# BoMingZhao/GaussianPrediction

Hardware: AMD Instinct MI355X
Metric: rendered views/s (full train step) @1M Gaussians 1352x1014 (higher is better)
Workload: dtype f32; 1 GPU; configs[2]: HyperNeRF-like 1M Gaussians, 1352x1014, stage-3 full train step (deform, raster, L1+SSIM loss, Adam: all HIP kernels); gaussians=1000000, width=1352, height=1014, keypoints=250, nearest_num=6, parallelism=view-parallel x1, ranks_seen_by_rccl=1, self_launched=False

## Files before the change

### gaussianprediction_amd/csrc/raster_kernels.hip

```cpp
#include "gp_common.h"
#include "raster_kernels.h"

#define GP_LOG2E 1.4426950408889634f
__device__ static const float SH_C0 = 0.28209479177387814f;
__device__ static const float SH_C1 = 0.4886025119029199f;
__device__ static const float SH_C2[5] = {1.0925484305920792f, -1.0925484305920792f, 0.31539156525252005f,
                                          -1.0925484305920792f, 0.5462742152960396f};
__device__ static const float SH_C3[7] = {-0.5900435899266435f, 2.890611442640554f, -0.4570457994644658f,
                                          0.3731763325901154f, -0.4570457994644658f, 1.445305721320277f,
                                          -0.5900435899266435f};

__device__ __forceinline__ float3 xform4x3(const float* __restrict__ m, float x, float y, float z) {
    float3 o;
    o.x = fmaf(m[0], x, fmaf(m[4], y, fmaf(m[8], z, m[12])));
    o.y = fmaf(m[1], x, fmaf(m[5], y, fmaf(m[9], z, m[13])));
    o.z = fmaf(m[2], x, fmaf(m[6], y, fmaf(m[10], z, m[14])));
    return o;
}
__device__ __forceinline__ float4 xform4x4(const float* __restrict__ m, float x, float y, float z) {
    float4 o;
    o.x = fmaf(m[0], x, fmaf(m[4], y, fmaf(m[8], z, m[12])));
    o.y = fmaf(m[1], x, fmaf(m[5], y, fmaf(m[9], z, m[13])));
    o.z = fmaf(m[2], x, fmaf(m[6], y, fmaf(m[10], z, m[14])));
    o.w = fmaf(m[3], x, fmaf(m[7], y, fmaf(m[11], z, m[15])));
// ... 853 lines not shown
                        if (MODE == 2) ++n_eval;
                        const int off = (int)lst[i];
                        const float4 q0 = *(const float4*)(s_rec + off);
                        const float4 q1 = *(const float4*)(s_rec + off + 16);
                        const float2 q2 = *(const float2*)(s_rec + off + 32);
                        const float dx = q0.x - pxf, dy = q0.y - pyf;
                        const float e = fmaf(dx, fmaf(q0.z, dx, q0.w * dy), fmaf(q1.x * dy, dy, q1.y));
                        if (!(e > q1.y)) {
                            const float alpha = fminf(0.99f, __builtin_amdgcn_exp2f(e));
                            if (!(alpha < 1.f / 255.f)) {
                                const float w = alpha * T;
                                const float test_T = T - w;
                                if (test_T < 0.0001f) {
                                    lim = -1;
                                } else {
                                    const int posv = off + sbase;
                                    C01.x = fmaf(q1.z, w, C01.x);
                                    C01.y = fmaf(q1.w, w, C01.y);
                                    C2D.x = fmaf(q2.x, w, C2D.x);
                                    C2D.y = fmaf(q2.y, w, C2D.y);
                                    if (w > best) { best = w; best_pos = posv; }
                                    T = test_T;
                                    last = posv;
                                    if (MODE == 2) ++n_contr;
                                }
                            }
                        }
                    }
                }
            }
            if (!__any(lim >= 0) && lane == 0) s_done[wave] = 1;
        }
    }
    if (MODE == 2) {
#pragma unroll
        for (int dd = 32; dd >= 1; dd >>= 1) { n_eval += __shfl_xor(n_eval, dd); n_contr += __shfl_xor(n_contr, dd); }
        if (lane == 0) { atomicAdd(&g_pair_counters[0], (unsigned long long)n_contr); atomicAdd(&g_pair_counters[1], (unsigned long long)n_eval); }
    }
    const float C0 = C01.x, C1 = C01.y, C2 = C2D.x, Dp = C2D.y;
    const size_t HW = (size_t)d.H * d.W;
    const int last_n = last < 0 ? 0 : last / CF2_REC + 1;
    if (inside) {
        const size_t pix = (size_t)py * d.W + px;
        out_color[pix] = fmaf(T, bg[0], C0);
        out_color[HW + pix] = fmaf(T, bg[1], C1);
        out_color[2 * HW + pix] = fmaf(T, bg[2], C2);
        out_depth[pix] = Dp;
        out_tidx[pix] = best_pos < 0 ? -1 : (int32_t)point_list[range.x + best_pos / CF2_REC];
        final_T[pix] = T;
        n_contrib[pix] = last_n;
    }
    if (tile_work) {
        int mx = inside ? last_n : 0;
#pragma unroll
        for (int dd = 32; dd >= 1; dd >>= 1) mx = max(mx, __shfl_xor(mx, dd));
        if (lane == 0) s_last[wave] = mx;
        __syncthreads();
        if (tid == 0) tile_work[tile] = max(max(s_last[0], s_last[1]), max(s_last[2], s_last[3]));
    }
}
__global__ __launch_bounds__(CF_THREADS) void gp_composite_fwd_sb_kernel(GP_CF_ARGS) {
    gp_composite_fwd_sb_body<1>(d, ranges, point_list, rec, bg, out_color, out_depth, out_tidx, final_T, n_contrib, order, tile_work, smask);
}
__global__ __launch_bounds__(CF_THREADS) void gp_composite_fwd_sbc_kernel(GP_CF_ARGS) {
    gp_composite_fwd_sb_body<0>(d, ranges, point_list, rec, bg, out_color, out_depth, out_tidx, final_T, n_contrib, order, tile_work, smask);
}
__global__ __launch_bounds__(CF_THREADS) void gp_composite_fwd_count_kernel(GP_CF_ARGS) {
    gp_composite_fwd_sb_body<2>(d, ranges, point_list, rec, bg, out_color, out_depth, out_tidx, final_T, n_contrib, order, tile_work, smask);
}
int gp_pair_counters_read(unsigned long long* out4) {
    if (hipDeviceSynchronize() != hipSuccess) return 1;
    if (hipMemcpyFromSymbol(out4, HIP_SYMBOL(g_pair_counters), 4 * sizeof(unsigned long long)) != hipSuccess) return 1;
    unsigned long long z[4] = {0, 0, 0, 0};
    return hipMemcpyToSymbol(HIP_SYMBOL(g_pair_counters), z, sizeof(z)) == hipSuccess ? 0 : 1;
}

__device__ __forceinline__ void dpp_scan2_add(float& a, float& b) {
    asm volatile(
        "s_nop 1\n\t"
        "v_add_f32_dpp %0, %0, %0 row_shr:1 row_mask:0xf bank_mask:0xf\n\t"
        "v_add_f32_dpp %1, %1, %1 row_shr:1 row_mask:0xf bank_mask:0xf\n\t"
        "s_nop 0\n\t"
        "v_add_f32_dpp %0, %0, %0 row_shr:2 row_mask:0xf bank_mask:0xf\n\t"
        "v_add_f32_dpp %1, %1, %1 row_shr:2 row_mask:0xf bank_mask:0xf\n\t"
        "s_nop 0\n\t"
        "v_add_f32_dpp %0, %0, %0 row_shr:4 row_mask:0xf bank_mask:0xf\n\t"
        "v_add_f32_dpp %1, %1, %1 row_shr:4 row_mask:0xf bank_mask:0xf\n\t"
        "s_nop 0\n\t"
        "v_add_f32_dpp %0, %0, %0 row_shr:8 row_mask:0xf bank_mask:0xf\n\t"
        "v_add_f32_dpp %1, %1, %1 row_shr:8 row_mask:0xf bank_mask:0xf\n\t"
        "s_nop 0\n\t"
        "v_add_f32_dpp %0, %0, %0 row_bcast:15 row_mask:0xa bank_mask:0xf\n\t"
        "v_add_f32_dpp %1, %1, %1 row_bcast:15 row_mask:0xa bank_mask:0xf\n\t"
        "s_nop 0\n\t"
        "v_add_f32_dpp %0, %0, %0 row_bcast:31 row_mask:0xc bank_mask:0xf\n\t"
        "v_add_f32_dpp %1, %1, %1 row_bcast:31 row_mask:0xc bank_mask:0xf\n\t"
        "s_nop 1"
        : "+v"(a), "+v"(b));
}
__device__ __forceinline__ void dpp_scan2_mul(float& a, float& b) {
    asm volatile(
        "s_nop 1\n\t"
        "v_mul_f32_dpp %0, %0, %0 row_shr:1 row_mask:0xf bank_mask:0xf\n\t"
        "v_mul_f32_dpp %1, %1, %1 row_shr:1 row_mask:0xf bank_mask:0xf\n\t"
        "s_nop 0\n\t"
        "v_mul_f32_dpp %0, %0, %0 row_shr:2 row_mask:0xf bank_mask:0xf\n\t"
        "v_mul_f32_dpp %1, %1, %1 row_shr:2 row_mask:0xf bank_mask:0xf\n\t"
        "s_nop 0\n\t"
        "v_mul_f32_dpp %0, %0, %0 row_shr:4 row_mask:0xf bank_mask:0xf\n\t"
        "v_mul_f32_dpp %1, %1, %1 row_shr:4 row_mask:0xf bank_mask:0xf\n\t"
        "s_nop 0\n\t"
        "v_mul_f32_dpp %0, %0, %0 row_shr:8 row_mask:0xf bank_mask:0xf\n\t"
        "v_mul_f32_dpp %1, %1, %1 row_shr:8 row_mask:0xf bank_mask:0xf\n\t"
        "s_nop 0\n\t"
        "v_mul_f32_dpp %0, %0, %0 row_bcast:15 row_mask:0xa bank_mask:0xf\n\t"
        "v_mul_f32_dpp %1, %1, %1 row_bcast:15 row_mask:0xa bank_mask:0xf\n\t"
        "s_nop 0\n\t"
        "v_mul_f32_dpp %0, %0, %0 row_bcast:31 row_mask:0xc bank_mask:0xf\n\t"
        "v_mul_f32_dpp %1, %1, %1 row_bcast:31 row_mask:0xc bank_mask:0xf\n\t"
        "s_nop 1"
        : "+v"(a), "+v"(b));
}



__device__ __forceinline__ void gp_pixpair(const RasterDims& d, int px0, int py, float bg0, float bg1, float bg2,
                                           const float* __restrict__ out_color, const float* __restrict__ out_depth,
                                           const float* __restrict__ final_T, const int32_t* __restrict__ n_contrib,
                                           const float* __restrict__ dL_dpix, const float* __restrict__ dL_dpixdepth, float4* o) {
    const size_t HW = (size_t)d.H * d.W;
    float dl[2][4] = {{0.f, 0.f, 0.f, 0.f}, {0.f, 0.f, 0.f, 0.f}};
    float tb[2] = {0.f, 0.f}, rem[2] = {0.f, 0.f};
    int nc[2] = {0, 0};
#pragma unroll
    for (int u = 0; u < 2; ++u) {
        const int px = px0 + u;
        if (px < d.W && py < d.H) {
            const size_t pix = (size_t)py * d.W + px;
            dl[u][0] = dL_dpix[pix]; dl[u][1] = dL_dpix[HW + pix]; dl[u][2] = dL_dpix[2 * HW + pix];
            dl[u][3] = dL_dpixdepth ? dL_dpixdepth[pix] : 0.f;
            tb[u] = final_T[pix] * (bg0 * dl[u][0] + bg1 * dl[u][1] + bg2 * dl[u][2]);
            rem[u] = out_color[pix] * dl[u][0] + out_color[HW + pix] * dl[u][1] + out_color[2 * HW + pix] * dl[u][2] - tb[u];
            if (dL_dpixdepth) rem[u] += out_depth[pix] * dl[u][3];
            nc[u] = n_contrib[pix];
        }
    }
    o[0] = make_float4(dl[0][0], dl[1][0], dl[0][1], dl[1][1]);
    o[1] = make_float4(dl[0][2], dl[1][2], tb[0], tb[1]);
    o[2] = make_float4(__int_as_float(nc[0]), __int_as_float(nc[1]), rem[0], rem[1]);
    o[3] = make_float4(dl[0][3], dl[1][3], 0.f, 0.f);
}

__device__ int g_bwd_ablate;
int gp_bwd_set_ablate(int v) { return hipMemcpyToSymbol(HIP_SYMBOL(g_bwd_ablate), &v, sizeof(int)) == hipSuccess ? 0 : 1; }

template <bool HAS_DEPTH, int ROWS, int COLS>
__device__ __forceinline__ void gp_composite_bwd_body(RasterDims d, const int2* __restrict__ ranges,
                                                       const uint32_t* __restrict__ point_list, const uint16_t* __restrict__ smask,
                                                       const float4* __restrict__ rec, const float* __restrict__ bg,
                                                       const float* __restrict__ out_color, const float* __restrict__ out_depth,
                                                       const float* __restrict__ final_T, const int32_t* __restrict__ n_contrib,
                                                       const float* __restrict__ dL_dpix, const float* __restrict__ dL_dpixdepth,
                                                       float* __restrict__ g_mean2D,
                                                       float* __restrict__ g_conic, float* __restrict__ g_opacity,
                                                       float* __restrict__ g_color, float* __restrict__ g_depth,
                                                       const uint32_t* __restrict__ order) {
    constexpr int PAIRS = ROWS * COLS / 2;
    static_assert(PAIRS <= 64, "one lane per pixel pair in the prologue");
    __shared__ float4 s_pp[PAIRS][4];
    __shared__ float2 s_dd[HAS_DEPTH ? PAIRS : 1];
    constexpr int parts_x = GP_TILE / COLS, parts = (GP_TILE / ROWS) * parts_x;
    const int xcd = blockIdx.x & 7, jw = blockIdx.x >> 3;
    const int slot = (jw / parts) * 8 + xcd;
    const int part = jw % parts;
    if (slot >= d.gx * d.gy) return;
    const int tile = __builtin_amdgcn_readfirstlane(order ? (int)order[slot] : slot);
    const int tx = tile % d.gx, ty = tile / d.gx;
    const int lane = threadIdx.x;
    const int2 range = ranges[tile];
    int max_nc;
    {
        max_nc = 0;
        if (lane < PAIRS) {
            float4 me[4];
            gp_pixpair(d, tx * GP_TILE + (part % parts_x) * COLS + 2 * (lane % (COLS / 2)), ty * GP_TILE + (part / parts_x) * ROWS + lane / (COLS / 2),
                       bg[0], bg[1], bg[2], out_color, out_depth, final_T, n_contrib, dL_dpix, HAS_DEPTH ? dL_dpixdepth : nullptr, me);
            const float4 t0 = me[0], t1 = me[1], t = me[2];
            s_pp[lane][1] = t0; s_pp[lane][2] = t1;
            s_pp[lane][0] = make_float4(t.x, t.y, 0.f, 0.f);
            if (HAS_DEPTH) { const float4 t3 = me[3]; s_dd[lane] = make_float2(t3.x, t3.y); }
            s_pp[lane][3] = make_float4(1.f, 1.f, t.z, t.w);
            max_nc = max(__float_as_int(t.x), __float_as_int(t.y));
        }
    }
#pragma unroll
    for (int dd = 32; dd >= 1; dd >>= 1) max_nc = max(max_nc, __shfl_xor(max_nc, dd));
    __builtin_amdgcn_wave_barrier();
    const float halfW = 0.5f * (float)d.W, halfH = 0.5f * (float)d.H;
    const int ablate = g_bwd_ablate;
    const int count = min(range.y - range.x, max_nc);
    const float px_base = (float)(tx * GP_TILE + (part % parts_x) * COLS), py_base = (float)(ty * GP_TILE + (part / parts_x) * ROWS);
    static_assert(ROWS == 8 && COLS == 8, "parts are the 8x8 quadrants: four sub-block bits of the saved 16-bit mask each");
    const uint32_t quad_bits = 0x33u << (8 * (part >> 1) + 2 * (part & 1));
    constexpr int QCAP = 448;
    __shared__ int2 s_q[QCAP];
    __shared__ float4 s_fl[3][64];
    __shared__ uint32_t s_flid[64];
    int qn = 0, src = 0;
    auto refill = [&]() {
        bool r[4];
        uint32_t ids[4], qm[4];
#pragma unroll
        for (int e = 0; e < 4; ++e) {
            const int k = src + 64 * e + lane;
            const int kk = range.x + (k < count ? k : count - 1);
            qm[e] = smask[kk];
            ids[e] = point_list[kk];
        }
        asm volatile("" ::"v"(qm[0]), "v"(qm[1]), "v"(qm[2]), "v"(qm[3]), "v"(ids[0]), "v"(ids[1]), "v"(ids[2]), "v"(ids[3]));
#pragma unroll
        for (int e = 0; e < 4; ++e) {
            const int k = src + 64 * e + lane;
            r[e] = k < count && (qm[e] & quad_bits) != 0u;
        }
#pragma unroll
        for (int e = 0; e < 4; ++e) {
            const unsigned long long bal = __ballot(r[e]);
            if (r[e]) s_q[qn + (int)gp_mbcnt(bal)] = make_int2(src + 64 * e + lane, (int)ids[e]);
            qn += (int)__popcll(bal);
        }
        src += 256;
    };
    while (qn < 128 && src < count) refill();
    __builtin_amdgcn_wave_barrier();
    float4 n0 = make_float4(0.f, 0.f, 0.f, 0.f), n1 = n0, n2 = n0;
    int2 ne = make_int2(0x7fffffff, 0);
    if (lane < qn) {
        ne = s_q[lane];
        n0 = rec[3 * (size_t)ne.y]; n1 = rec[3 * (size_t)ne.y + 1]; n2 = rec[3 * (size_t)ne.y + 2];
    }
    while (qn > 0) {
        const int nb = min(64, qn);
        const bool have = lane < nb;
        const int b0 = __builtin_amdgcn_readfirstlane(ne.x);
        const int pos = have ? ne.x : 0x7fffffff;
        const uint32_t id = (uint32_t)ne.y;
        const float4 q0 = n0, q1 = n1, q2 = n2;
        {
            int2 mv[6];
#pragma unroll
            for (int e = 0; e < 6; ++e) mv[e] = (64 + e * 64 + lane < qn) ? s_q[64 + e * 64 + lane] : make_int2(0, 0);
            __builtin_amdgcn_wave_barrier();
#pragma unroll
            for (int e = 0; e < 6; ++e) if (64 + e * 64 + lane < qn) s_q[e * 64 + lane] = mv[e];
            qn -= nb;
            __builtin_amdgcn_wave_barrier();
            while (qn < 128 && src < count) refill();
            __builtin_amdgcn_wave_barrier();
            n0 = make_float4(0.f, 0.f, 0.f, 0.f); n1 = n0; n2 = n0;
            ne = make_int2(0x7fffffff, 0);
            if (lane < qn) {
                ne = s_q[lane];
                n0 = rec[3 * (size_t)ne.y]; n1 = rec[3 * (size_t)ne.y + 1]; n2 = rec[3 * (size_t)ne.y + 2];
            }
        }
        const float As = q0.z, Bs = q0.w, Cs = q1.x;
        const float lop = have ? q1.y : -INFINITY, zdep = q1.z;
        const float opac = q2.w;
        const float LN2 = 0.6931471805599453f;
        const float cxx = -2.f * LN2 * q0.z, cxy = -LN2 * q0.w, cyy = -2.f * LN2 * q1.x;
        const v2f cr = {q2.x, q2.x}, cg = {q2.y, q2.y}, cb = {q2.z, q2.z};
        v2f a_op = {0.f, 0.f}, a_r = {0.f, 0.f}, a_g = {0.f, 0.f}, a_b = {0.f, 0.f}, a_d = {0.f, 0.f}, s_xx = {0.f, 0.f};
        float S_x = 0.f, S_y = 0.f, S_xy = 0.f, S_yy = 0.f;
        float any_m = 0.f;
        auto fma2 = [](v2f a, v2f b, v2f c) { return (v2f){fmaf(a.x, b.x, c.x), fmaf(a.y, b.y, c.y)}; };
        v2f dxs[COLS / 2];
#pragma unroll
        for (int cp = 0; cp < COLS / 2; ++cp) dxs[cp] = (v2f){q0.x - (px_base + (float)(2 * cp)), q0.x - (px_base + (float)(2 * cp + 1))};
#pragma unroll 1
        for (int row = 0; row < ((ablate & 2) ? 0 : ROWS); ++row) {
            const float dy = q0.y - (py_base + (float)row);
            const float tB = Bs * dy, uC = fmaf(Cs * dy, dy, lop);
            v2f r_h = {0.f, 0.f}, r_hx = {0.f, 0.f};
            if (!HAS_DEPTH) {
                const v2f As2 = {As, As}, tB2 = {tB, tB}, uC2 = {uC, uC};
                const v2f dx0 = dxs[0], dx1 = dxs[1], dx2 = dxs[2], dx3 = dxs[3];
                const uint32_t vpp = (uint32_t)(uintptr_t)&s_pp[row * (COLS / 2)][0];
                unsigned long long sv, c0, c1, t0;
#ifndef GP_CB_LADDER_NOPS
#define GP_CB_LADDER_NOPS 1
#endif
#if GP_CB_LADDER_NOPS
#define CB_NOP0 "s_nop 0\n\t"
#define CB_NOP1 "s_nop 1\n\t"
#else
#define CB_NOP0 ""
#define CB_NOP1 ""
#endif
#define CB_SCAN2(OPC, R0, R1)                                                                   \
    CB_NOP1                                                                                     \
    OPC " " R0 ", " R0 ", " R0 " row_shr:1 row_mask:0xf bank_mask:0xf\n\t"                       \
    OPC " " R1 ", " R1 ", " R1 " row_shr:1 row_mask:0xf bank_mask:0xf\n\t"                       \
    CB_NOP0                                                                                     \
    OPC " " R0 ", " R0 ", " R0 " row_shr:2 row_mask:0xf bank_mask:0xf\n\t"                       \
    OPC " " R1 ", " R1 ", " R1 " row_shr:2 row_mask:0xf bank_mask:0xf\n\t"                       \
    CB_NOP0                                                                                     \
    OPC " " R0 ", " R0 ", " R0 " row_shr:4 row_mask:0xf bank_mask:0xf\n\t"                       \
    OPC " " R1 ", " R1 ", " R1 " row_shr:4 row_mask:0xf bank_mask:0xf\n\t"                       \
    CB_NOP0                                                                                     \
    OPC " " R0 ", " R0 ", " R0 " row_shr:8 row_mask:0xf bank_mask:0xf\n\t"                       \
    OPC " " R1 ", " R1 ", " R1 " row_shr:8 row_mask:0xf bank_mask:0xf\n\t"                       \
    CB_NOP0                                                                                     \
    OPC " " R0 ", " R0 ", " R0 " row_bcast:15 row_mask:0xa bank_mask:0xf\n\t"                    \
    OPC " " R1 ", " R1 ", " R1 " row_bcast:15 row_mask:0xa bank_mask:0xf\n\t"                    \
    CB_NOP0                                                                                     \
    OPC " " R0 ", " R0 ", " R0 " row_bcast:31 row_mask:0xc bank_mask:0xf\n\t"                    \
    OPC " " R1 ", " R1 ", " R1 " row_bcast:31 row_mask:0xc bank_mask:0xf\n\t"                    \
    CB_NOP1
#define CB_STEP(CP, O0, O1, O2, O3, DX)                                                                               \
    "ds_read_b64 v[64:65], %[vpp] offset:" #O0 "\n\t"                                                                \
    "ds_read_b128 v[66:69], %[vpp] offset:" #O1 "\n\t"                                                               \
    "ds_read_b128 v[70:73], %[vpp] offset:" #O2 "\n\t"                                                               \
    "ds_read_b128 v[74:77], %[vpp] offset:" #O3 "\n\t"                                                               \
    "v_pk_fma_f32 v[78:79], %[As2], " DX ", %[tB2] op_sel_hi:[0,1,0]\n\t"                                             \
    "s_nop 0\n\t"                                                                                                   \
    "v_pk_fma_f32 v[78:79], " DX ", v[78:79], %[uC2] op_sel_hi:[1,1,0]\n\t"                                           \
    "s_waitcnt lgkmcnt(3)\n\t"                                                                                       \
    "v_max_i32 v80, v64, v65\n\t"                                                                                    \
    "v_cmp_lt_i32 vcc, %[b0], v80\n\t"                                                                               \
    "s_cbranch_vccz 9" #CP "f\n\t"                                                                                   \
    "v_exp_f32 v80, v78\n\t"                                    \
    "v_exp_f32 v81, v79\n\t"                                                                                         \
    "v_cmp_lt_i32 %[c0], %[pos], v64\n\t"                                                                            \
    "v_cmp_lt_i32 %[c1], %[pos], v65\n\t"                                                                            \
    "v_cmp_ngt_f32 %[t0], v78, %[lop]\n\t"                 \
    "s_and_b64 %[c0], %[c0], %[t0]\n\t"                                                                              \
    "v_cmp_ngt_f32 %[t0], v79, %[lop]\n\t"                                                                           \
    "s_and_b64 %[c1], %[c1], %[t0]\n\t"                                                                              \
    "v_cmp_ngt_f32 vcc, 0x3b808081, v80\n\t"            \
    "s_and_b64 %[c0], %[c0], vcc\n\t"                                                                                \
    "v_cmp_ngt_f32 vcc, 0x3b808081, v81\n\t"                                                                         \
    "s_and_b64 %[c1], %[c1], vcc\n\t"                                                                              \
    "s_or_b64 %[t0], %[c0], %[c1]\n\t"                                                                               \
    "s_cbranch_scc0 9" #CP "f\n\t"                                                                                   \
    "v_cndmask_b32 v80, 0, v80, %[c0]\n\t"            \
    "v_cndmask_b32 v81, 0, v81, %[c1]\n\t"                                                                           \
    "v_min_f32 v82, 0x3f7d70a4, v80\n\t"                                                                             \
    "v_min_f32 v83, 0x3f7d70a4, v81\n\t"                                                                             \
    "v_max3_f32 %[any], %[any], v82, v83\n\t"                                                                        \
    "v_pk_add_f32 v[84:85], v[82:83], 1.0 op_sel_hi:[1,0] neg_lo:[1,0] neg_hi:[1,0]\n\t"                              \
    "s_waitcnt lgkmcnt(0)\n\t"                                                                                       \
    "v_pk_mul_f32 v[86:87], %[cb], v[70:71]\n\t"                                                                     \
    "v_rcp_f32 v88, v84\n\t"                                                                                         \
    "v_rcp_f32 v89, v85\n\t"                                                                                         \
    "v_pk_fma_f32 v[86:87], %[cg], v[68:69], v[86:87]\n\t"                                                           \
    CB_SCAN2("v_mul_f32_dpp", "v84", "v85")                                                                           \
    "v_pk_fma_f32 v[86:87], %[cr], v[66:67], v[86:87]\n\t"                                                           \
    "v_pk_mul_f32 v[90:91], v[74:75], v[84:85]\n\t"                                                                  \
    "s_nop 0\n\t"                                                                                                   \
    "v_pk_mul_f32 v[84:85], v[90:91], v[88:89]\n\t"                                                                  \
    "s_nop 0\n\t"                                                                                                   \
    "v_pk_mul_f32 v[94:95], v[82:83], v[84:85]\n\t"                                                                  \
    "s_nop 0\n\t"                                                                                                   \
    "v_pk_mul_f32 v[96:97], v[94:95], v[86:87]\n\t"                                                                  \
    CB_SCAN2("v_add_f32_dpp", "v96", "v97")                                                                           \
    "v_pk_add_f32 v[92:93], v[76:77], v[96:97] neg_lo:[0,1] neg_hi:[0,1]\n\t"                                         \
    "s_bfm_b64 exec, 1, 63\n\t"                                                                                      \
    "ds_write_b128 %[vpp], v[90:93] offset:" #O3 "\n\t"                                                              \
    "s_mov_b64 exec, %[sv]\n\t"                                                                                      \
    "v_pk_add_f32 v[96:97], v[92:93], v[72:73]\n\t"                                                                  \
    "v_pk_fma_f32 %[a_r], v[94:95], v[66:67], %[a_r]\n\t"                                                            \
    "v_pk_mul_f32 v[96:97], v[96:97], v[88:89]\n\t"                                                                  \
    "v_pk_fma_f32 %[a_g], v[94:95], v[68:69], %[a_g]\n\t"                                                            \
    "v_pk_fma_f32 v[96:97], v[84:85], v[86:87], v[96:97] neg_lo:[0,0,1] neg_hi:[0,0,1]\n\t"                           \
    "v_pk_fma_f32 %[a_b], v[94:95], v[70:71], %[a_b]\n\t"                                                            \
    "v_pk_mul_f32 v[96:97], v[80:81], v[96:97]\n\t"                                                                  \
    "s_nop 0\n\t"                                                                                                   \
    "v_pk_add_f32 %[a_op], %[a_op], v[96:97]\n\t"                 \
    "v_pk_add_f32 %[r_h], %[r_h], v[96:97]\n\t"                                                                      \
    "v_pk_mul_f32 v[96:97], v[96:97], " DX "\n\t"                                                                    \
    "s_nop 0\n\t"                                                                                                   \
    "v_pk_add_f32 %[r_hx], %[r_hx], v[96:97]\n\t"                                                                    \
    "v_pk_fma_f32 %[s_xx], v[96:97], " DX ", %[s_xx]\n\t"                                                            \
    "9" #CP ":\n\t"
                asm volatile(
                    "s_mov_b64 %[sv], exec\n\t"
                    CB_STEP(0, 0, 16, 32, 48, "%[dx0]")
                    CB_STEP(1, 64, 80, 96, 112, "%[dx1]")
                    CB_STEP(2, 128, 144, 160, 176, "%[dx2]")
                    CB_STEP(3, 192, 208, 224, 240, "%[dx3]")
                    : [a_op] "+v"(a_op), [a_r] "+v"(a_r), [a_g] "+v"(a_g), [a_b] "+v"(a_b), [s_xx] "+v"(s_xx), [r_h] "+v"(r_h), [r_hx] "+v"(r_hx),
                      [any] "+v"(any_m), [sv] "=&s"(sv), [c0] "=&s"(c0), [c1] "=&s"(c1), [t0] "=&s"(t0)
                    : [As2] "v"(As2), [tB2] "v"(tB2), [uC2] "v"(uC2), [lop] "v"(lop), [cr] "v"(cr), [cg] "v"(cg), [cb] "v"(cb), [dx0] "v"(dx0),
                      [dx1] "v"(dx1), [dx2] "v"(dx2), [dx3] "v"(dx3), [pos] "v"(pos), [vpp] "v"(vpp), [b0] "s"(b0)
                    : "vcc", "scc", "memory", "v64", "v65", "v66", "v67", "v68", "v69", "v70", "v71", "v72", "v73", "v74", "v75", "v76", "v77",
                      "v78", "v79", "v80", "v81", "v82", "v83", "v84", "v85", "v86", "v87", "v88", "v89", "v90", "v91", "v92", "v93", "v94",
                      "v95", "v96", "v97");
#undef CB_STEP
#undef CB_SCAN2
            } else
#pragma unroll
            for (int cp = 0; cp < COLS / 2; ++cp) {
                const int pr = row * (COLS / 2) + cp;
                const float4 ncf = s_pp[pr][0];
                const int2 nc = make_int2(__float_as_int(ncf.x), __float_as_int(ncf.y));
                const float4 v0 = s_pp[pr][1], v1 = s_pp[pr][2], cy = s_pp[pr][3];
                float2 v3 = make_float2(0.f, 0.f);
                if (HAS_DEPTH) v3 = s_dd[pr];
                const v2f dx = dxs[cp];
                const v2f pw = {fmaf(dx.x, fmaf(As, dx.x, tB), uC), fmaf(dx.y, fmaf(As, dx.y, tB), uC)};
                const v2f E = {__builtin_amdgcn_exp2f(pw.x), __builtin_amdgcn_exp2f(pw.y)};
                const int ncx = nc.x, ncy = nc.y;
                if (max(ncx, ncy) > b0) {
                    const bool c0 = (pos < ncx) && !(pw.x > lop) && !(E.x < 1.f / 255.f);
                    const bool c1 = (pos < ncy) && !(pw.y > lop) && !(E.y < 1.f / 255.f);
                    if (__builtin_amdgcn_ballot_w64(c0 || c1) != 0ull) {
                        const v2f Em = {c0 ? E.x : 0.f, c1 ? E.y : 0.f};
                        const v2f am = {fminf(0.99f, Em.x), fminf(0.99f, Em.y)};
                        any_m = fmaxf(any_m, fmaxf(am.x, am.y));
                        const v2f om = 1.f - am;
                        v2f cdot = cb * (v2f){v1.x, v1.y};
                        cdot = fma2(cg, (v2f){v0.z, v0.w}, cdot);
                        cdot = fma2(cr, (v2f){v0.x, v0.y}, cdot);
                        v2f dLd = {0.f, 0.f};
                        if (HAS_DEPTH) { dLd.x = v3.x; dLd.y = v3.y; cdot = fma2((v2f){zdep, zdep}, dLd, cdot); }
                        const v2f rom = {__builtin_amdgcn_rcpf(om.x), __builtin_amdgcn_rcpf(om.y)};
                        float il0 = om.x, il1 = om.y;
                        dpp_scan2_mul(il0, il1);
                        const v2f Tnext = (v2f){cy.x, cy.y} * (v2f){il0, il1};
                        const v2f Tj = Tnext * rom;
                        const v2f w = am * Tj;
                        const v2f sv = w * cdot;
                        float is0 = sv.x, is1 = sv.y;
                        dpp_scan2_add(is0, is1);
                        const v2f rem = {cy.z, cy.w};
                        const v2f tbv = {v1.z, v1.w};
                        const v2f suffix = rem - (v2f){is0, is1};
                        const v2f dL_dalpha = fma2(Tj, cdot, -((suffix + tbv) * rom));
                        a_r = fma2(w, (v2f){v0.x, v0.y}, a_r);
                        a_g = fma2(w, (v2f){v0.z, v0.w}, a_g);
                        a_b = fma2(w, (v2f){v1.x, v1.y}, a_b);
                        if (HAS_DEPTH) a_d = fma2(w, dLd, a_d);
                        const v2f h = Em * dL_dalpha;
                        a_op += h;
                        const v2f hx = h * dx;
                        r_h += h;
                        r_hx += hx;
                        s_xx = fma2(hx, dx, s_xx);
                        if (lane == 63) s_pp[pr][3] = make_float4(Tnext.x, Tnext.y, cy.z - is0, cy.w - is1);
                    }
                }
            }
            {
                const float rh = r_h.x + r_h.y, rhx = r_hx.x + r_hx.y;
                S_x += rhx;
                S_y = fmaf(dy, rh, S_y);
                S_xy = fmaf(dy, rhx, S_xy);
                S_yy = fmaf(dy * dy, rh, S_yy);
            }
        }
        {
            const bool mine = have && any_m > 0.f;
            float* fl = (float*)&s_fl[0][0];
            float* fm = (float*)&s_fl[1][0];
            float* fh = (float*)&s_fl[2][0];
            const float S_xx = s_xx.x + s_xx.y;
            const float g_mx = -(cxx * S_x + cxy * S_y), g_my = -(cyy * S_y + cxy * S_x);
            ((float4*)fl)[lane] = make_float4(g_mx * halfW, g_my * halfH, -0.5f * S_xx, -S_xy);
            ((float4*)fm)[lane] = make_float4(-0.5f * S_yy, mine ? (a_op.x + a_op.y) / opac : 0.f, a_r.x + a_r.y, a_g.x + a_g.y);
            ((float4*)fh)[lane] = make_float4(a_b.x + a_b.y, HAS_DEPTH ? a_d.x + a_d.y : 0.f, 0.f, 0.f);
            s_flid[lane] = mine ? id : 0xffffffffu;
            __builtin_amdgcn_wave_barrier();
            const int comp = lane & 15, sub = lane >> 4;
            const float* src_c = comp < 4 ? fl : (comp < 8 ? fm : fh);
            if (comp < (HAS_DEPTH ? 10 : 9)) {
#pragma unroll 4
                for (int r = 0; r < 16; ++r) {
                    const int sp = r * 4 + sub;
                    const uint32_t gid = s_flid[sp];
                    if (gid != 0xffffffffu && !(ablate & 1)) atomicAdd(&g_mean2D[GP_ACC_STRIDE * (size_t)gid + comp], src_c[sp * 4 + (comp & 3)]);
                }
            }
        }
        __builtin_amdgcn_wave_barrier();
    }
}
__global__ __launch_bounds__(64) void gp_composite_bwd_kernel(GP_CB_ARGS) {
    gp_composite_bwd_body<false, GP_BWD_ROWS, GP_BWD_COLS>(d, ranges, point_list, smask, rec, bg, out_color, out_depth, final_T, n_contrib, dL_dpix, dL_dpixdepth, g_mean2D, g_conic, g_opacity, g_color, g_depth, order);
}
__global__ __launch_bounds__(64) void gp_composite_bwd_depth_kernel(GP_CB_ARGS) {
    gp_composite_bwd_body<true, GP_BWD_ROWS, GP_BWD_COLS>(d, ranges, point_list, smask, rec, bg, out_color, out_depth, final_T, n_contrib, dL_dpix, dL_dpixdepth, g_mean2D, g_conic, g_opacity, g_color, g_depth, order);
}

constexpr int SHA_Y = 45, SHA_G = 60, SHA_ROW = 63;

template <int NT>
__device__ __forceinline__ void adam_unstage_sh(const float* s_sh, const AdamFuseDev& af, size_t off, int nblk, int tid, int lim) {
    constexpr int CH = NT * 4;
    const int total = nblk * 45;
    float* __restrict__ p = af.p_rest + off; float* __restrict__ m = af.m_rest + off; float* __restrict__ v = af.v_rest + off;
    auto update = [&](int idx, float& pp, float& mm, float& vq) {
        const int gi = idx / 45, k = idx - gi * 45;
        const float* row = s_sh + gi * SHA_ROW;
        const float g = k < lim ? row[SHA_Y + k / 3] * row[SHA_G + k % 3] : 0.f;
        pp = row[k];
        gp_adam_update(pp, g, mm, vq, af.b1, af.b2, af.eps, af.step_rest, af.bc2_sqrt);
    };
    constexpr int AU = 6;
    for (int e = tid * 4; e < total; e += AU * CH) {
        float4 mv[AU], vv[AU];
#pragma unroll
        for (int c = 0; c < AU; ++c) {
            const int ec = e + CH * c, el = ec + 3 < total ? ec : 0;
            mv[c] = *(const float4*)(m + el); vv[c] = *(const float4*)(v + el);
        }
#pragma unroll
        for (int c = 0; c < AU; ++c) {
            const int ec = e + CH * c;
            if (ec + 3 < total) {
                float4 pv;
                float* pp = (float*)&pv; float* mm = (float*)&mv[c]; float* vq = (float*)&vv[c];
#pragma unroll
                for (int u = 0; u < 4; ++u) update(ec + u, pp[u], mm[u], vq[u]);
                *(float4*)(p + ec) = pv; *(float4*)(m + ec) = mv[c]; *(float4*)(v + ec) = vv[c];
            } else {
                for (int idx = ec; idx < total; ++idx) update(idx, p[idx], m[idx], v[idx]);
            }
        }
    }
}

__device__ __forceinline__ void sh_basis(int D, float x, float y, float z, float* Y) {
#pragma unroll
    for (int k = 0; k < 16; ++k) Y[k] = 0.f;
    if (D > 0) {
        Y[1] = -SH_C1 * y;
        Y[2] = SH_C1 * z;
        Y[3] = -SH_C1 * x;
        if (D > 1) {
            const float xx = x * x, yy = y * y, zz = z * z, xy = x * y, yz = y * z, xz = x * z;
            Y[4] = SH_C2[0] * xy;
            Y[5] = SH_C2[1] * yz;
            Y[6] = SH_C2[2] * (2.f * zz - xx - yy);
            Y[7] = SH_C2[3] * xz;
            Y[8] = SH_C2[4] * (xx - yy);
            if (D > 2) {
                Y[9] = SH_C3[0] * y * (3.f * xx - yy);
                Y[10] = SH_C3[1] * xy * z;
                Y[11] = SH_C3[2] * y * (4.f * zz - xx - yy);
                Y[12] = SH_C3[3] * z * (2.f * zz - 3.f * xx - 3.f * yy);
                Y[13] = SH_C3[4] * x * (4.f * zz - xx - yy);
                Y[14] = SH_C3[5] * z * (xx - yy);
                Y[15] = SH_C3[6] * x * (xx - 3.f * yy);
            }
        }
    }
}

template <int SH_MODE, bool SH_ADAM = false>
__device__ __forceinline__ void preprocess_bwd_body(
    RasterDims d, const float* __restrict__ means3D, const float* __restrict__ scales, const float* __restrict__ rotations,
    const float* __restrict__ shs, const float* __restrict__ shs_rest, const float* __restrict__ cov3D_precomp,
    const float* __restrict__ view, const float* __restrict__ proj, const float* __restrict__ campos,
    const int32_t* __restrict__ radii, const uint8_t* __restrict__ clamped, const float* __restrict__ g_mean2D,
    const float* __restrict__ g_conic, const float* __restrict__ g_opacity, const float* __restrict__ g_color,
    const float* __restrict__ g_depth, float* __restrict__ dL_dmeans3D, float* __restrict__ dL_dmeans2D,
    float* __restrict__ dL_dshs, float* __restrict__ dL_dshs_rest, float* __restrict__ dL_dcolors,
    float* __restrict__ dL_dopacities, float* __restrict__ dL_dscales, float* __restrict__ dL_drots,
    float* __restrict__ dL_dcov3D, int accumulate_shs, AdamFuseDev af) {
    static_assert(!SH_ADAM || SH_MODE == 2, "the fused SH Adam step is the split layout's");
    constexpr int NT = SH_ADAM ? GP_PB_ADAM_THREADS : 256, NG = SH_ADAM ? GP_PB_ADAM_GAUSSIANS : 256;
    __shared__ float s_sh[SH_MODE == 0 ? 1 : NG * (SH_ADAM ? SHA_ROW : 49)];
    const int tid = threadIdx.x;
    const int base = blockIdx.x * NG;
    const int i = tid < NG ? base + tid : d.N;
    const int nblk = min(NG, d.N - base);
    const bool use_sh = dL_dcolors == nullptr;
    constexpr int SROW = SH_ADAM ? SHA_ROW : SH_MODE == 1 ? 49 : 45;
    constexpr int SOFF = SH_MODE == 1 ? 0 : 3;
    float dsh_dc[3] = {0.f, 0.f, 0.f};
    const int ii = i < d.N ? i : d.N - 1;
    const int rad_i = radii[ii];
    const float4* accl = (const float4*)(g_mean2D + GP_ACC_STRIDE * (size_t)ii);
    const float4 A0 = accl[0], A1 = accl[1], A2 = accl[2];
    const float px = means3D[3 * ii], py = means3D[3 * ii + 1], pz = means3D[3 * ii + 2];
    float sc3[3] = {0.f, 0.f, 0.f}, q4[4] = {0.f, 0.f, 0.f, 0.f};
    if (!cov3D_precomp) {
#pragma unroll
        for (int k = 0; k < 3; ++k) sc3[k] = scales[3 * ii + k];
#pragma unroll
        for (int k = 0; k < 4; ++k) q4[k] = rotations[4 * ii + k];
    }
    const float raw_o = d.raw_opacity ? d.raw_opacity[ii] : 0.f;
    const uint8_t cl = dL_dcolors ? (uint8_t)0 : clamped[ii];
    const float acc_mean2D[2] = {A0.x, A0.y}, acc_conic[3] = {A0.z, A0.w, A1.x}, acc_opacity = A1.y,
                acc_color[3] = {A1.z, A1.w, A2.x}, acc_depth = A2.y;
    if (SH_MODE != 0) {
        if (SH_ADAM) {
            stage_sh<45, SHA_ROW, NT>(s_sh, shs_rest + (size_t)base * 45, nblk, tid);
        } else if (use_sh && d.D > 0) {
            if (SH_MODE == 1) stage_sh<48>(s_sh, shs + (size_t)base * 48, nblk, tid);
            if (SH_MODE == 2) stage_sh<45>(s_sh, shs_rest + (size_t)base * 45, nblk, tid);
        }
        __syncthreads();
    }
    do {
    if (i >= d.N) break;
    const bool vis = rad_i > 0;
    dL_dmeans2D[3 * i] = vis ? acc_mean2D[0] : 0.f;
    dL_dmeans2D[3 * i + 1] = vis ? acc_mean2D[1] : 0.f;
    dL_dmeans2D[3 * i + 2] = 0.f;
    {
        const float go = vis ? acc_opacity : 0.f;
        float out = go;
        if (d.raw_opacity) {
            const float so = 1.f / (1.f + expf(-raw_o));
            out = go * 1.f * so * (1.f - so);
        }
        dL_dopacities[i] = out;
    }
    const float3 pv = xform4x3(view, px, py, pz);
    float c6[6];
    if (cov3D_precomp) {
#pragma unroll
        for (int k = 0; k < 6; ++k) c6[k] = cov3D_precomp[6 * i + k];
    } else {
        if (d.raw_opacity) {
#pragma unroll
            for (int k = 0; k < 3; ++k) sc3[k] = expf(sc3[k]);
        }
        compute_cov3D(sc3, d.scale_mod, q4, c6);
    }
    float abc[3];
    ProjCtx cx;
    compute_cov2D(pv, d.fx, d.fy, d.tanfovx, d.tanfovy, c6, view, abc, &cx);
    const float a = abc[0] + 0.3f, b = abc[1], c = abc[2] + 0.3f;
    const float det = a * c - b * b;
    const float gA = acc_conic[0], gB = acc_conic[1], gC = acc_conic[2];
// ... 197 lines not shown
```

Before: 922.6 views/s.

## Use ring-buffer splat queue and skip finished pixel rows in composite backward

Replaces the shift-down compaction of the shared splat queue with a circular head/tail ring buffer, removing per-batch LDS copies of up to 384 queue entries. It also computes a per-batch ballot of which pixel pairs are still live (n_contrib above the batch start), so rows whose pairs are all finished are skipped entirely. Individual pair steps in the hand-written assembly branch on a scalar bit instead of a vector compare. A compile-time counter instrumentation path (GP_CB_COUNT) is added but disabled by default. The risks are extra modulo arithmetic on queue indices and a slightly smaller queue capacity.

```diff
diff --git a/gaussianprediction_amd/csrc/raster_kernels.hip b/gaussianprediction_amd/csrc/raster_kernels.hip
--- a/gaussianprediction_amd/csrc/raster_kernels.hip
+++ b/gaussianprediction_amd/csrc/raster_kernels.hip
@@ -1029,7 +1029,24 @@
 }
 
 __device__ int g_bwd_ablate;
+#ifndef GP_CB_COUNT
 int gp_bwd_set_ablate(int v) { return hipMemcpyToSymbol(HIP_SYMBOL(g_bwd_ablate), &v, sizeof(int)) == hipSuccess ? 0 : 1; }
+#define CB_COUNT(i, n) ((void)0)
+#else
+constexpr int CB_NCOUNT = 13;
+__device__ unsigned long long g_cb_count[CB_NCOUNT];
+int gp_bwd_set_ablate(int v) {
+    static const char* names[CB_NCOUNT] = {"waves", "waves_with_work", "batches", "refills", "rows_walked", "rows_dead", "steps_executed",
+                                           "steps_skipped_pair_finished", "steps_skipped_no_lane", "flushes_with_lanes", "flushes_empty",
+                                           "flush_lanes", "queued_instances"};
+    unsigned long long h[CB_NCOUNT], z[CB_NCOUNT] = {};
+    if (hipDeviceSynchronize() != hipSuccess || hipMemcpyFromSymbol(h, HIP_SYMBOL(g_cb_count), sizeof(h)) != hipSuccess) return 1;
+    for (int i = 0; i < CB_NCOUNT; ++i) fprintf(stderr, "[cb_count] %-28s %14llu   per wave %10.3f\n", names[i], h[i], h[0] ? (double)h[i] / (double)h[0] : 0.0);
+    if (hipMemcpyToSymbol(HIP_SYMBOL(g_cb_count), z, sizeof(z)) != hipSuccess) return 1;
+    return hipMemcpyToSymbol(HIP_SYMBOL(g_bwd_ablate), &v, sizeof(int)) == hipSuccess ? 0 : 1;
+}
+#define CB_COUNT(i, n) (cbc[i] += (n))
+#endif
 
 template <bool HAS_DEPTH, int ROWS, int COLS>
 __device__ __forceinline__ void gp_composite_bwd_body(RasterDims d, const int2* __restrict__ ranges,
@@ -1056,6 +1073,7 @@
     const int lane = threadIdx.x;
     const int2 range = ranges[tile];
     int max_nc;
+    int pair_nc;
     {
         max_nc = 0;
         if (lane < PAIRS) {
@@ -1069,22 +1087,28 @@
             s_pp[lane][3] = make_float4(1.f, 1.f, t.z, t.w);
             max_nc = max(__float_as_int(t.x), __float_as_int(t.y));
         }
+        pair_nc = max_nc;
     }
 #pragma unroll
     for (int dd = 32; dd >= 1; dd >>= 1) max_nc = max(max_nc, __shfl_xor(max_nc, dd));
     __builtin_amdgcn_wave_barrier();
     const float halfW = 0.5f * (float)d.W, halfH = 0.5f * (float)d.H;
     const int ablate = g_bwd_ablate;
-    const int count = min(range.y - range.x, max_nc);
+    const int count = __builtin_amdgcn_readfirstlane(min(range.y - range.x, max_nc));
     const float px_base = (float)(tx * GP_TILE + (part % parts_x) * COLS), py_base = (float)(ty * GP_TILE + (part / parts_x) * ROWS);
     static_assert(ROWS == 8 && COLS == 8, "parts are the 8x8 quadrants: four sub-block bits of the saved 16-bit mask each");
     const uint32_t quad_bits = 0x33u << (8 * (part >> 1) + 2 * (part & 1));
-    constexpr int QCAP = 448;
+    constexpr int QCAP = 384;
     __shared__ int2 s_q[QCAP];
     __shared__ float4 s_fl[3][64];
     __shared__ uint32_t s_flid[64];
-    int qn = 0, src = 0;
+    int qn = 0, qh = 0, qt = 0, src = 0;
+    auto qwrap = [](int i) { return i >= QCAP ? i - QCAP : i; };
+#ifdef GP_CB_COUNT
+    unsigned cbc[CB_NCOUNT] = {};
+#endif
     auto refill = [&]() {
+        CB_COUNT(3, 1);
         bool r[4];
         uint32_t ids[4], qm[4];
 #pragma unroll
@@ -1103,13 +1127,16 @@
 #pragma unroll
         for (int e = 0; e < 4; ++e) {
             const unsigned long long bal = __ballot(r[e]);
-            if (r[e]) s_q[qn + (int)gp_mbcnt(bal)] = make_int2(src + 64 * e + lane, (int)ids[e]);
-            qn += (int)__popcll(bal);
+            if (r[e]) s_q[qwrap(qt + (int)gp_mbcnt(bal))] = make_int2(src + 64 * e + lane, (int)ids[e]);
+            const int c = (int)__popcll(bal);
+            qn += c;
+            qt = qwrap(qt + c);
         }
         src += 256;
     };
     while (qn < 128 && src < count) refill();
     __builtin_amdgcn_wave_barrier();
+    CB_COUNT(0, 1); CB_COUNT(1, qn > 0 ? 1 : 0);
     float4 n0 = make_float4(0.f, 0.f, 0.f, 0.f), n1 = n0, n2 = n0;
     int2 ne = make_int2(0x7fffffff, 0);
     if (lane < qn) {
@@ -1123,21 +1150,17 @@
         const int pos = have ? ne.x : 0x7fffffff;
         const uint32_t id = (uint32_t)ne.y;
         const float4 q0 = n0, q1 = n1, q2 = n2;
+        CB_COUNT(2, 1); CB_COUNT(12, nb);
         {
-            int2 mv[6];
-#pragma unroll
-            for (int e = 0; e < 6; ++e) mv[e] = (64 + e * 64 + lane < qn) ? s_q[64 + e * 64 + lane] : make_int2(0, 0);
-            __builtin_amdgcn_wave_barrier();
-#pragma unroll
-            for (int e = 0; e < 6; ++e) if (64 + e * 64 + lane < qn) s_q[e * 64 + lane] = mv[e];
             qn -= nb;
+            qh = qwrap(qh + nb);
             __builtin_amdgcn_wave_barrier();
             while (qn < 128 && src < count) refill();
             __builtin_amdgcn_wave_barrier();
             n0 = make_float4(0.f, 0.f, 0.f, 0.f); n1 = n0; n2 = n0;
             ne = make_int2(0x7fffffff, 0);
             if (lane < qn) {
-                ne = s_q[lane];
+                ne = s_q[qwrap(qh + lane)];
                 n0 = rec[3 * (size_t)ne.y]; n1 = rec[3 * (size_t)ne.y + 1]; n2 = rec[3 * (size_t)ne.y + 2];
             }
         }
@@ -1154,12 +1177,21 @@
         v2f dxs[COLS / 2];
 #pragma unroll
         for (int cp = 0; cp < COLS / 2; ++cp) dxs[cp] = (v2f){q0.x - (px_base + (float)(2 * cp)), q0.x - (px_base + (float)(2 * cp + 1))};
+        const uint32_t live = (uint32_t)__ballot(pair_nc > b0);
 #pragma unroll 1
         for (int row = 0; row < ((ablate & 2) ? 0 : ROWS); ++row) {
+            const uint32_t rb = (live >> (row * (COLS / 2))) & ((1u << (COLS / 2)) - 1u);
+            if (rb == 0u) { CB_COUNT(5, 1); continue; }
+            CB_COUNT(4, 1);
             const float dy = q0.y - (py_base + (float)row);
             const float tB = Bs * dy, uC = fmaf(Cs * dy, dy, lop);
             v2f r_h = {0.f, 0.f}, r_hx = {0.f, 0.f};
-            if (!HAS_DEPTH) {
+#ifdef GP_CB_COUNT
+            constexpr bool hand = false;
+#else
+            constexpr bool hand = !HAS_DEPTH;
+#endif
+            if (hand) {
                 const v2f As2 = {As, As}, tB2 = {tB, tB}, uC2 = {uC, uC};
                 const v2f dx0 = dxs[0], dx1 = dxs[1], dx2 = dxs[2], dx3 = dxs[3];
                 const uint32_t vpp = (uint32_t)(uintptr_t)&s_pp[row * (COLS / 2)][0];
@@ -1195,6 +1227,8 @@
     OPC " " R1 ", " R1 ", " R1 " row_bcast:31 row_mask:0xc bank_mask:0xf\n\t"                    \
     CB_NOP1
 #define CB_STEP(CP, O0, O1, O2, O3, DX)                                                                               \
+    "s_bitcmp1_b32 %[rb], " #CP "\n\t"                 \
+    "s_cbranch_scc0 9" #CP "f\n\t"                                                                                   \
     "ds_read_b64 v[64:65], %[vpp] offset:" #O0 "\n\t"                                                                \
     "ds_read_b128 v[66:69], %[vpp] offset:" #O1 "\n\t"                                                               \
     "ds_read_b128 v[70:73], %[vpp] offset:" #O2 "\n\t"                                                               \
@@ -1203,13 +1237,10 @@
     "s_nop 0\n\t"                                                                                                   \
     "v_pk_fma_f32 v[78:79], " DX ", v[78:79], %[uC2] op_sel_hi:[1,1,0]\n\t"                                           \
     "s_waitcnt lgkmcnt(3)\n\t"                                                                                       \
-    "v_max_i32 v80, v64, v65\n\t"                                                                                    \
-    "v_cmp_lt_i32 vcc, %[b0], v80\n\t"                                                                               \
-    "s_cbranch_vccz 9" #CP "f\n\t"                                                                                   \
+    "v_cmp_lt_i32 %[c0], %[pos], v64\n\t"                                                                            \
+    "v_cmp_lt_i32 %[c1], %[pos], v65\n\t"                                                                            \
     "v_exp_f32 v80, v78\n\t"                                    \
     "v_exp_f32 v81, v79\n\t"                                                                                         \
-    "v_cmp_lt_i32 %[c0], %[pos], v64\n\t"                                                                            \
-    "v_cmp_lt_i32 %[c1], %[pos], v65\n\t"                                                                            \
     "v_cmp_ngt_f32 %[t0], v78, %[lop]\n\t"                 \
     "s_and_b64 %[c0], %[c0], %[t0]\n\t"                                                                              \
     "v_cmp_ngt_f32 %[t0], v79, %[lop]\n\t"                                                                           \
@@ -1269,7 +1300,7 @@
                     : [a_op] "+v"(a_op), [a_r] "+v"(a_r), [a_g] "+v"(a_g), [a_b] "+v"(a_b), [s_xx] "+v"(s_xx), [r_h] "+v"(r_h), [r_hx] "+v"(r_hx),
                       [any] "+v"(any_m), [sv] "=&s"(sv), [c0] "=&s"(c0), [c1] "=&s"(c1), [t0] "=&s"(t0)
                     : [As2] "v"(As2), [tB2] "v"(tB2), [uC2] "v"(uC2), [lop] "v"(lop), [cr] "v"(cr), [cg] "v"(cg), [cb] "v"(cb), [dx0] "v"(dx0),
-                      [dx1] "v"(dx1), [dx2] "v"(dx2), [dx3] "v"(dx3), [pos] "v"(pos), [vpp] "v"(vpp), [b0] "s"(b0)
+                      [dx1] "v"(dx1), [dx2] "v"(dx2), [dx3] "v"(dx3), [pos] "v"(pos), [vpp] "v"(vpp), [rb] "s"(rb)
                     : "vcc", "scc", "memory", "v64", "v65", "v66", "v67", "v68", "v69", "v70", "v71", "v72", "v73", "v74", "v75", "v76", "v77",
                       "v78", "v79", "v80", "v81", "v82", "v83", "v84", "v85", "v86", "v87", "v88", "v89", "v90", "v91", "v92", "v93", "v94",
                       "v95", "v96", "v97");
@@ -1279,19 +1310,21 @@
 #pragma unroll
             for (int cp = 0; cp < COLS / 2; ++cp) {
                 const int pr = row * (COLS / 2) + cp;
-                const float4 ncf = s_pp[pr][0];
-                const int2 nc = make_int2(__float_as_int(ncf.x), __float_as_int(ncf.y));
-                const float4 v0 = s_pp[pr][1], v1 = s_pp[pr][2], cy = s_pp[pr][3];
-                float2 v3 = make_float2(0.f, 0.f);
-                if (HAS_DEPTH) v3 = s_dd[pr];
-                const v2f dx = dxs[cp];
-                const v2f pw = {fmaf(dx.x, fmaf(As, dx.x, tB), uC), fmaf(dx.y, fmaf(As, dx.y, tB), uC)};
-                const v2f E = {__builtin_amdgcn_exp2f(pw.x), __builtin_amdgcn_exp2f(pw.y)};
-                const int ncx = nc.x, ncy = nc.y;
-                if (max(ncx, ncy) > b0) {
+                if ((rb >> cp) & 1u) {
+                    const float4 ncf = s_pp[pr][0];
+                    const int2 nc = make_int2(__float_as_int(ncf.x), __float_as_int(ncf.y));
+                    const float4 v0 = s_pp[pr][1], v1 = s_pp[pr][2], cy = s_pp[pr][3];
+                    float2 v3 = make_float2(0.f, 0.f);
+                    if (HAS_DEPTH) v3 = s_dd[pr];
+                    const v2f dx = dxs[cp];
+                    const v2f pw = {fmaf(dx.x, fmaf(As, dx.x, tB), uC), fmaf(dx.y, fmaf(As, dx.y, tB), uC)};
+                    const v2f E = {__builtin_amdgcn_exp2f(pw.x), __builtin_amdgcn_exp2f(pw.y)};
+                    const int ncx = nc.x, ncy = nc.y;
                     const bool c0 = (pos < ncx) && !(pw.x > lop) && !(E.x < 1.f / 255.f);
                     const bool c1 = (pos < ncy) && !(pw.y > lop) && !(E.y < 1.f / 255.f);
+                    CB_COUNT(8, __builtin_amdgcn_ballot_w64(c0 || c1) == 0ull ? 1 : 0);
                     if (__builtin_amdgcn_ballot_w64(c0 || c1) != 0ull) {
+                        CB_COUNT(6, 1);
                         const v2f Em = {c0 ? E.x : 0.f, c1 ? E.y : 0.f};
                         const v2f am = {fminf(0.99f, Em.x), fminf(0.99f, Em.y)};
                         any_m = fmaxf(any_m, fmaxf(am.x, am.y));
@@ -1326,6 +1359,8 @@
                         s_xx = fma2(hx, dx, s_xx);
                         if (lane == 63) s_pp[pr][3] = make_float4(Tnext.x, Tnext.y, cy.z - is0, cy.w - is1);
                     }
+                } else {
+                    CB_COUNT(7, 1);
                 }
             }
             {
@@ -1338,6 +1373,7 @@
         }
         {
             const bool mine = have && any_m > 0.f;
+            CB_COUNT(9, __ballot(mine) != 0ull ? 1 : 0); CB_COUNT(10, __ballot(mine) != 0ull ? 0 : 1); CB_COUNT(11, (int)__popcll(__ballot(mine)));
             float* fl = (float*)&s_fl[0][0];
             float* fm = (float*)&s_fl[1][0];
             float* fh = (float*)&s_fl[2][0];
@@ -1361,6 +1397,10 @@
         }
         __builtin_amdgcn_wave_barrier();
     }
+#ifdef GP_CB_COUNT
+    if (lane == 0)
+        for (int i = 0; i < CB_NCOUNT; ++i) if (cbc[i]) atomicAdd(&g_cb_count[i], (unsigned long long)cbc[i]);
+#endif
 }
 __global__ __launch_bounds__(64) void gp_composite_bwd_kernel(GP_CB_ARGS) {
     gp_composite_bwd_body<false, GP_BWD_ROWS, GP_BWD_COLS>(d, ranges, point_list, smask, rec, bg, out_color, out_depth, final_T, n_contrib, dL_dpix, dL_dpixdepth, g_mean2D, g_conic, g_opacity, g_color, g_depth, order);
```

After: 931.1 views/s (median of 6 runs). Within noise of the previous version (+0.9%).
